# yml-bit/CTA-GAN

Hardware: AMD Instinct MI355X
Metric: paired 512x512 slices/sec (G+D step); generator rel-L2 vs CPU reference (higher is better)
Workload: dtype bf16; 1 GPU; HdGan stage-2 full G+D train step (G, Reg, STN, D_m, losses, Adam x3), 16 paired 512x512 slices/GPU; per_gpu_batch=16, global_batch=16, size=512, parallelism=single, rccl_ranks=1, dp_backend=none

## Files before the change

### cta_gan_amd/csrc/conv_dispatch.h

```cpp
#pragma once
#include "common.h"
#include "ctg_knobs.h"

static inline int tap_dy(int tw) { return (tw & 0xff) - 64; }
static inline int tap_dx(int tw) { return ((tw >> 8) & 0xff) - 64; }

struct TapWindow {
    int dymin = 127, dymax = -128, dxmin = 127, dxmax = -128;
    void add(int dy, int dx) {
        dymin = dy < dymin ? dy : dymin; dymax = dy > dymax ? dy : dymax;
        dxmin = dx < dxmin ? dx : dxmin; dxmax = dx > dxmax ? dx : dxmax;
    }
    int kh() const { return dymax - dymin + 1; }
    int kw() const { return dxmax - dxmin + 1; }
    int dy0() const { return dymin; }
    int dx0() const { return dxmin; }
};
static inline TapWindow tap_window(const int* taps, int ntaps) {
    TapWindow w;
    for (int t = 0; t < ntaps; ++t) w.add(tap_dy(taps[t]), tap_dx(taps[t]));
    return w;
}

static inline bool taps_3x3(const int* taps, bool flipped) {
    for (int t = 0; t < 9; ++t) {
        const int dy = t / 3 - 1, dx = t % 3 - 1;
        if (tap_dy(taps[t]) != (flipped ? -dy : dy) || tap_dx(taps[t]) != (flipped ? -dx : dx)) return false;
    }
    return true;
}
static inline bool taps_conv3x3_s2(const int* taps) {
    for (int t = 0; t < 9; ++t)
        if ((taps[t] >> 16) != t) return false;
    return taps_3x3(taps, false);
}
static inline bool taps_convT3x3_classes(const int* c_ntaps, const int* c_oy0, const int* c_ox0, const int* c_tap0, const int* taps) {
    static const int want_n[4] = {1, 2, 2, 4}, want_oy[4] = {0, 0, 1, 1}, want_ox[4] = {0, 1, 0, 1};
    static const int want_t[9][3] = {{0, 0, 4}, {0, 1, 3}, {0, 0, 5}, {1, 0, 1}, {0, 0, 7}, {1, 1, 0}, {1, 0, 2}, {0, 1, 6}, {0, 0, 8}};
    int t = 0;
    for (int q = 0; q < 4; ++q) {
        if (c_ntaps[q] != want_n[q] || c_oy0[q] != want_oy[q] || c_ox0[q] != want_ox[q] || c_tap0[q] != t) return false;
        for (int k = 0; k < want_n[q]; ++k, ++t)
            if (tap_dy(taps[t]) != want_t[t][0] || tap_dx(taps[t]) != want_t[t][1] || (taps[t] >> 16) != want_t[t][2]) return false;
    }
    return true;
}

struct BandPlan { int band_rows, nbands; };
static inline BandPlan band_plan(int rows, int min_band, long slots, long strips, int band_env) {
    long nb = slots / strips;
    if (nb < 1) nb = 1;
    int band = (int)((rows + nb - 1) / nb);
    if (band < min_band) band = min_band;
    if (band_env >= 8) band = band_env;
    return BandPlan{band, (rows + band - 1) / band};
}

template <auto Kernel, typename Args>
static int launch_lds(dim3 grid, dim3 block, int smem, hipStream_t st, const Args& s) {
    static unsigned long long attr_mask = 0;
    const int rc = ctg_lds_attr_once((const void*)Kernel, smem, &attr_mask);
    if (rc != CTG_OK) return rc;
    hipLaunchKernelGGL(Kernel, grid, block, smem, st, s);
    return ctg_launch_status();
}

static inline bool halo_th8(int Hs, int Ws, int Cout, int B, int ncls) {
    const long wgs = (long)((Hs + 15) / 16) * ((Ws + 15) / 16) * ((Cout + 127) / 128) * B;
    return !ctg_knobs().no_th8 && ncls != 4 && Hs >= 16 && wgs < ctg_knobs().th8_wgs;
}
```

### cta_gan_amd/csrc/conv_halo.h

```cpp
#pragma once
#include <stdlib.h>
#include <type_traits>
#include "common.h"
#include "conv_dispatch.h"

struct ConvArgs {
    const void* x;
    const void* w;
    void* y;
    const float* bias;
    int B, Hi, Wi, Cin, x_ld;
    int Ho, Wo, Cout, y_ld;
    int Hs, Ws, oy0, ox0, os, is;
    int frame;
    int pad_mode, act;
    int w_tap_stride;
    int ntaps;
    int taps[64];
    int kh, kw, dy0, dx0;
    float* stats;
    const void* res;
    const void* fold;
    int res_ld, fold_ld;
    const void* bz;
    const float* bmean;
    const float* brstd;
    float* bstats;
    int bz_ld, bact;
    int ncls;
    int s2d;
    int pair_lo;
    unsigned long long* nie_sync;
    int nie_act;
    int nie_budget;
    int c_ntaps[4], c_tap0[4], c_oy0[4], c_ox0[4], c_kh[4], c_kw[4], c_dy0[4], c_dx0[4];
};

typedef const __attribute__((address_space(1))) void* gptr_t;
typedef __attribute__((address_space(3))) void* lptr_t;

extern __device__ __attribute__((aligned(16))) unsigned g_zero_chunk[4];

__device__ __forceinline__ void unpack_bf16x8(const u32x4 t, float (&f)[8]) {
#pragma unroll
    for (int i = 0; i < 4; ++i) {
        f[2 * i] = __uint_as_float(t[i] << 16);
        f[2 * i + 1] = __uint_as_float(t[i] & 0xffff0000u);
    }
}
__device__ __forceinline__ void add_bf16x8(float (&f)[8], const bf16_t* p) {
    const u32x4 t = *reinterpret_cast<const u32x4*>(p);
#pragma unroll
    for (int i = 0; i < 4; ++i) {
        f[2 * i] += __uint_as_float(t[i] << 16);
        f[2 * i + 1] += __uint_as_float(t[i] & 0xffff0000u);
    }
}

#define CONV_ACT_RT (-1)
template <int ACT> __device__ __forceinline__ float act_apply_c(float x, int act) {
    if constexpr (ACT == ACT_NONE) return x;
    else if constexpr (ACT == ACT_RELU) return x > 0.f ? x : 0.f;
    else if constexpr (ACT == ACT_LRELU) return x > 0.f ? x : LRELU_SLOPE * x;
    else return act_apply(x, act);
}
template <typename F> __device__ __forceinline__ void act_switch(int act, F&& f) {
    if (act == ACT_NONE) f(std::integral_constant<int, ACT_NONE>{});
    else if (act == ACT_RELU) f(std::integral_constant<int, ACT_RELU>{});
    else if (act == ACT_LRELU) f(std::integral_constant<int, ACT_LRELU>{});
    else f(std::integral_constant<int, CONV_ACT_RT>{});
}
struct GradMask {
    float slope;
    unsigned keep;
    __device__ __forceinline__ explicit GradMask(int bact)
        : slope(bact == ACT_LRELU ? LRELU_SLOPE : 1.f), keep(bact == ACT_RELU ? 0u : 0xffffffffu) {}
    __device__ __forceinline__ float apply(float g, float xh) const {
        return xh > 0.f ? g : __uint_as_float(__float_as_uint(slope * g) & keep);
    }
};

template <int N, bool V1_FIRST> __device__ __forceinline__ float pinned_sumsq(const float (&v)[N]) {
#pragma clang fp contract(off)
    if constexpr (N == 1) {
        return v[0] * v[0];
    } else {
        float s = V1_FIRST ? __fmaf_rn(v[0], v[0], v[1] * v[1]) : __fmaf_rn(v[1], v[1], v[0] * v[0]);
#pragma unroll
        for (int k = 2; k < N; ++k) s = __fmaf_rn(v[k], v[k], s);
        return s;
    }
}

#define HALO_W 16

template <typename T, typename OutT, int BN, int WM, int WN, int KCH, int ABUF, int TH, bool FUSE, int KWC, bool MC = false, bool PK = false,
          bool S2D = false, bool NIE = false>
__global__ __launch_bounds__(WM * WN * 64, ((TH / WM) * (BN / (WN * 16)) > 16 ? 2 : 4))
void conv_halo_kernel(const ConvArgs a) {
    static_assert(!NIE || (!MC && !S2D && sizeof(T) == 2 && !std::is_same<OutT, float>::value),
                  "InstanceNorm in the epilogue: plain bf16 / split-pair launches");
    static_assert(!S2D || (!MC && !FUSE && KWC == 0 && ABUF == 1), "polyphase K walk: plain single-buffer instantiations");
    static_assert(!PK || (KCH == 8 && sizeof(T) == 2), "split-pair K steps: [hi 32 | lo 32] rows of bf16");
    constexpr int NTH = WM * WN * 64;
    constexpr int EPC = VecOf<T>::N;
    constexpr int BKE = KCH * EPC;
    constexpr int BM = TH * HALO_W;
    constexpr int TM = TH / WM;
    static_assert(TH % WM == 0, "tile rows per wave");
    constexpr int TN = BN / (WN * 16);
    constexpr int B_CH = BN * KCH;
    constexpr int B_IT = (B_CH + NTH - 1) / NTH;
    static_assert(B_CH % 64 == 0, "weight tile");
    extern __shared__ __attribute__((aligned(16))) char smem[];

    const int tid = threadIdx.x, lane = tid & 63, wave = __builtin_amdgcn_readfirstlane(tid >> 6);
    const int wm = wave / WN, wn = wave % WN;
    const int n = blockIdx.y;
    const int ntn = (a.Cout + BN - 1) / BN;
    const int id = xcd_contiguous(blockIdx.x, gridDim.x);
    const int n0 = (id % ntn) * BN;
    const int spc = id / ntn;
    int sp = spc, kh_ = a.kh, kw_ = a.kw, dy0 = a.dy0, dx0 = a.dx0, ntaps = a.ntaps, tap0 = 0, oy0_ = a.oy0, ox0_ = a.ox0;
    if constexpr (MC) {
        const int q = spc & 3;
        sp = spc >> 2;
        kh_ = a.c_kh[q]; kw_ = a.c_kw[q]; dy0 = a.c_dy0[q]; dx0 = a.c_dx0[q];
        ntaps = a.c_ntaps[q]; tap0 = a.c_tap0[q]; oy0_ = a.c_oy0[q]; ox0_ = a.c_ox0[q];
    }
    const int HPW = KWC ? HALO_W + KWC - 1 : HALO_W + kw_ - 1, HPH = TH + kh_ - 1;
    const int HPC = HPH * HPW * KCH;
    const int HPC64 = (HPC + 63) & ~63;
    const int nchunk = a.Cin / BKE;
    const int nbufA = (nchunk > 1 && ABUF == 2) ? 2 : 1;
    char* sA = smem;
    char* sB = smem + nbufA * HPC64 * 16;

    const int tx_n = (a.Ws + HALO_W - 1) / HALO_W;
    const int y0 = (sp / tx_n) * TH, x0 = (sp % tx_n) * HALO_W;
    const T* __restrict__ X = (const T*)a.x + (size_t)n * a.Hi * a.Wi * a.x_ld;
    const T* __restrict__ W = (const T*)a.w;

    const int h_it = (HPC64 + NTH - 1) / NTH;
    const unsigned hpw_magic = (unsigned)((0x100000000ULL + HPW - 1) / HPW);
    const int Hi = a.Hi, Wi = a.Wi, x_ld = a.x_ld, pad_mode = a.pad_mode;
    const int iy00 = y0 + dy0, ix00 = x0 + dx0;
    constexpr bool PRE = (KWC >= 3) && !MC;
    constexpr int H_PRE = PRE ? ((((TH + KWC - 1) * (HALO_W + KWC - 1) * KCH + 63) & ~63) + NTH - 1) / NTH : 1;
    int hoff[H_PRE];
    if constexpr (PRE) {
#pragma unroll
        for (int it = 0; it < H_PRE; ++it) {
            const int sl = tid + NTH * it;
            const int hrow = sl / KCH;
            const int hy = (int)__umulhi((unsigned)hrow, hpw_magic), hx = hrow - hy * HPW;
            const int kc = swz<KCH>(hx, sl % KCH);
            int iy = iy00 + hy, ix = ix00 + hx;
            if (pad_mode == PAD_REFLECT) {
                iy = reflect_idx(iy, Hi);
                ix = reflect_idx(ix, Wi);
            }
            const bool ok = (sl < HPC) && ((unsigned)iy < (unsigned)Hi) && ((unsigned)ix < (unsigned)Wi);
            hoff[it] = ok ? (iy * Wi + ix) * x_ld + (PK ? (kc & 3) * EPC + (kc >> 2) * a.pair_lo : kc * EPC) : -1;
        }
    }
    int phy = S2D ? a.c_oy0[0] : 0, phx = S2D ? a.c_ox0[0] : 0;
    auto issue_halo = [&](int it, int buf, int kc0) __attribute__((always_inline)) {
        if constexpr (PRE) {
#pragma unroll
            for (int j = 0; j < H_PRE; ++j) {
                if (j == it && NTH * j + 64 * wave < HPC64) {
                    const T* src = hoff[j] >= 0 ? X + (hoff[j] + kc0) : (const T*)g_zero_chunk;
                    __builtin_amdgcn_global_load_lds((gptr_t)src, (lptr_t)(sA + (buf * HPC64 + NTH * j + 64 * wave) * 16), 16, 0, 0);
                }
            }
        } else
        if (NTH * it + 64 * wave < HPC64) {
            const int sl = tid + NTH * it;
            const int hrow = sl / KCH;
            const int hy = (int)__umulhi((unsigned)hrow, hpw_magic), hx = hrow - hy * HPW;
            const int kc = swz<KCH>(hx, sl % KCH);
            int iy = iy00 + hy, ix = ix00 + hx;
            if constexpr (S2D) { iy = 2 * iy + phy; ix = 2 * ix + phx; }
            if (pad_mode == PAD_REFLECT) {
                iy = reflect_idx(iy, Hi);
                ix = reflect_idx(ix, Wi);
            }
            const bool ok = (sl < HPC) && ((unsigned)iy < (unsigned)Hi) && ((unsigned)ix < (unsigned)Wi);
            const T* src = ok ? X + ((iy * Wi + ix) * x_ld + (PK ? (kc & 3) * EPC + (kc >> 2) * a.pair_lo : kc * EPC) + kc0)
                              : (const T*)g_zero_chunk;
            __builtin_amdgcn_global_load_lds((gptr_t)src, (lptr_t)(sA + (buf * HPC64 + NTH * it + 64 * wave) * 16), 16, 0, 0);
        }
    };
    int boff[B_IT];
    const bool b_active = (B_CH % NTH == 0) || (tid < B_CH);
#pragma unroll
    for (int it = 0; it < B_IT; ++it) {
        const int s = (tid + NTH * it) % B_CH;
        const int row = s / KCH;
        boff[it] = (n0 + row) * a.Cin + swz<KCH>(row, s % KCH) * EPC;
    }
    const int w_tap_stride = a.w_tap_stride;
    auto issue_w = [&](int buf, int tw, int kc0) __attribute__((always_inline)) {
        if (b_active) {
            const int wbase = (tw >> 16) * w_tap_stride + kc0;
#pragma unroll
            for (int it = 0; it < B_IT; ++it)
                if (B_CH % NTH == 0 || NTH * it + 64 * wave < B_CH)
                    __builtin_amdgcn_global_load_lds((gptr_t)(W + wbase + boff[it]),
                                                     (lptr_t)(sB + (buf * B_CH + NTH * it + 64 * wave) * 16), 16, 0, 0);
        }
    };

    f32x4 acc[TM][TN];
#pragma unroll
    for (int i = 0; i < TM; ++i)
#pragma unroll
        for (int j = 0; j < TN; ++j) acc[i][j] = f32x4{0.f, 0.f, 0.f, 0.f};

    const int wo0 = (((wn * TN) * 16 + (lane & 15)) * KCH + swz<KCH>(lane & 15, lane >> 4)) * 16;
    auto compute = [&](int abuf, int bbuf, int tw) __attribute__((always_inline)) {
        const char* pa = sA + abuf * HPC64 * 16;
        const char* pb = sB + bbuf * B_CH * 16;
        const int ky = (tw & 0xff) - 64 - dy0, kx = ((tw >> 8) & 0xff) - 64 - dx0;
        const int hx = kx + (lane & 15);
        const char* prow = pa + (ky + wm * TM) * (HPW * KCH * 16);
        const int xo0 = (hx * KCH + swz<KCH>(hx, lane >> 4)) * 16;
        if constexpr (PK) {
            u32x4 fa[TM], fb[TN], fl[TN];
#pragma unroll
            for (int mt = 0; mt < TM; ++mt) fa[mt] = *reinterpret_cast<const u32x4*>(prow + xo0 + mt * (HPW * KCH * 16));
#pragma unroll
            for (int nt = 0; nt < TN; ++nt) fb[nt] = *reinterpret_cast<const u32x4*>(pb + wo0 + nt * (16 * KCH * 16));
#pragma unroll
            for (int mt = 0; mt < TM; ++mt)
#pragma unroll
                for (int nt = 0; nt < TN; ++nt)
                    acc[mt][nt] = __builtin_amdgcn_mfma_f32_16x16x32_bf16(
                        __builtin_bit_cast(bf16x8, fb[nt]), __builtin_bit_cast(bf16x8, fa[mt]), acc[mt][nt], 0, 0, 0);
#pragma unroll
            for (int nt = 0; nt < TN; ++nt) fl[nt] = *reinterpret_cast<const u32x4*>(pb + (wo0 ^ 64) + nt * (16 * KCH * 16));
#pragma unroll
            for (int mt = 0; mt < TM; ++mt)
#pragma unroll
                for (int nt = 0; nt < TN; ++nt)
                    acc[mt][nt] = __builtin_amdgcn_mfma_f32_16x16x32_bf16(
                        __builtin_bit_cast(bf16x8, fl[nt]), __builtin_bit_cast(bf16x8, fa[mt]), acc[mt][nt], 0, 0, 0);
#pragma unroll
            for (int mt = 0; mt < TM; ++mt) fa[mt] = *reinterpret_cast<const u32x4*>(prow + (xo0 ^ 64) + mt * (HPW * KCH * 16));
#pragma unroll
            for (int mt = 0; mt < TM; ++mt)
#pragma unroll
                for (int nt = 0; nt < TN; ++nt)
                    acc[mt][nt] = __builtin_amdgcn_mfma_f32_16x16x32_bf16(
                        __builtin_bit_cast(bf16x8, fb[nt]), __builtin_bit_cast(bf16x8, fa[mt]), acc[mt][nt], 0, 0, 0);
        } else
#pragma unroll
        for (int ks = 0; ks < KCH / 4; ++ks) {
            u32x4 fa[TM], fb[TN];
            const int xo = xo0 ^ (ks * 64), wo = wo0 ^ (ks * 64);
#pragma unroll
            for (int mt = 0; mt < TM; ++mt)
                fa[mt] = *reinterpret_cast<const u32x4*>(prow + xo + mt * (HPW * KCH * 16));
#pragma unroll
            for (int nt = 0; nt < TN; ++nt)
                fb[nt] = *reinterpret_cast<const u32x4*>(pb + wo + nt * (16 * KCH * 16));
#pragma unroll
            for (int mt = 0; mt < TM; ++mt)
#pragma unroll
                for (int nt = 0; nt < TN; ++nt) {
                    if constexpr (sizeof(T) == 2) {
                        acc[mt][nt] = __builtin_amdgcn_mfma_f32_16x16x32_bf16(
                            __builtin_bit_cast(bf16x8, fb[nt]), __builtin_bit_cast(bf16x8, fa[mt]), acc[mt][nt], 0, 0, 0);
                    } else {
                        const f32x4 va = __builtin_bit_cast(f32x4, fa[mt]);
                        const f32x4 vb = __builtin_bit_cast(f32x4, fb[nt]);
#pragma unroll
                        for (int q = 0; q < 4; ++q)
                            acc[mt][nt] = __builtin_amdgcn_mfma_f32_16x16x4f32(vb[q], va[q], acc[mt][nt], 0, 0, 0);
                    }
                }
        }
    };

    const bool wave_rows_valid = y0 + wm * TM < a.Hs;
    const int pps = (h_it + ntaps - 1) / ntaps;
    auto issue_halo_all = [&](int buf, int kc0) __attribute__((always_inline)) {
        if constexpr (PRE) {
#pragma unroll
            for (int j = 0; j < H_PRE; ++j)
                if (NTH * j + 64 * wave < HPC64) {
                    const T* src = hoff[j] >= 0 ? X + (hoff[j] + kc0) : (const T*)g_zero_chunk;
                    __builtin_amdgcn_global_load_lds((gptr_t)src, (lptr_t)(sA + (buf * HPC64 + NTH * j + 64 * wave) * 16), 16, 0, 0);
                }
        } else {
            for (int it = 0; it < h_it; ++it) issue_halo(it, buf, kc0);
        }
    };
    auto xslice = [&](int cc) __attribute__((always_inline)) { return PK ? cc * (BKE / 2) : cc * BKE; };
    if constexpr (S2D) { ntaps = a.c_ntaps[0]; tap0 = a.c_tap0[0]; }
    issue_halo_all(0, 0);
    int tw_cur = a.taps[tap0];
    issue_w(0, tw_cur, 0);
    __syncthreads();
    int S = nchunk * ntaps;
    if constexpr (S2D) {
        S = 0;
        for (int q = 0; q < a.ncls; ++q) S += nchunk * a.c_ntaps[q];
    }
    const int nslices = S2D ? nchunk * a.ncls : nchunk;
    int c = 0, t = 0;
    for (int s = 0; s < S; ++s) {
        int tn = t + 1, cn = c;
        if (tn == ntaps) { tn = 0; cn = c + 1; }
        int tw_next = 0;
        int ntaps_n = ntaps, tap0_n = tap0;
        if constexpr (S2D) {
            if (cn != c && cn < nslices) { const int q = cn / nchunk; ntaps_n = a.c_ntaps[q]; tap0_n = a.c_tap0[q]; }
        }
        if (s + 1 < S) {
            tw_next = a.taps[tap0_n + tn];
            issue_w((s + 1) & 1, tw_next, (S2D ? cn % nchunk : cn) * BKE);
        }
        if (ABUF == 2 && c + 1 < nchunk) {
            for (int q = 0; q < pps; ++q) {
                const int it = t * pps + q;
                if (it < h_it) issue_halo(it, (c + 1) & 1, xslice(c + 1));
            }
        }
        if (wave_rows_valid) compute(nbufA == 2 ? (c & 1) : 0, s & 1, tw_cur);
        __syncthreads();
        if (ABUF == 1 && cn != c && cn < nslices) {
            if constexpr (S2D) { const int q = cn / nchunk; phy = a.c_oy0[q]; phx = a.c_ox0[q]; }
            issue_halo_all(0, xslice(S2D ? cn % nchunk : cn));
            __syncthreads();
        }
        t = tn;
        c = cn;
        ntaps = ntaps_n;
        tap0 = tap0_n;
        tw_cur = tw_next;
    }

    const int co_l = (lane >> 4) * 4;
    if (a.stats != nullptr) {
        float* red = reinterpret_cast<float*>(smem);
#pragma unroll
        for (int nt = 0; nt < TN; ++nt) {
            float s1[4] = {0.f, 0.f, 0.f, 0.f}, s2[4], vq[4][TM];
#pragma unroll
            for (int mt = 0; mt < TM; ++mt) {
                const bool valid = (y0 + wm * TM + mt < a.Hs) && (x0 + (lane & 15) < a.Ws);
#pragma unroll
                for (int r = 0; r < 4; ++r) {
                    const float v = valid ? acc[mt][nt][r] : 0.f;
                    s1[r] += v;
                    vq[r][mt] = v;
                }
            }
#pragma unroll
            for (int r = 0; r < 4; ++r) s2[r] = pinned_sumsq<TM, KWC == 3 && !(FUSE && std::is_same<OutT, bfpair_t>::value)>(vq[r]);
#pragma unroll
            for (int r = 0; r < 4; ++r) {
                s1[r] = row16_sum_to_lane15(s1[r]);
                s2[r] = row16_sum_to_lane15(s2[r]);
                if ((lane & 15) == 15) {
                    const int cl = (wn * TN + nt) * 16 + co_l + r;
                    red[(wm * BN + cl) * 2] = s1[r];
                    red[(wm * BN + cl) * 2 + 1] = s2[r];
                }
            }
        }
        __syncthreads();
        const int ntile = gridDim.x / ntn;
        for (int cl = tid; cl < BN; cl += NTH) {
            if (n0 + cl < a.Cout) {
                float t1 = 0.f, t2 = 0.f;
#pragma unroll
                for (int w = 0; w < WM; ++w) { t1 += red[(w * BN + cl) * 2]; t2 += red[(w * BN + cl) * 2 + 1]; }
                float* dst = a.stats + (((size_t)n * ntile + spc) * a.Cout + n0 + cl) * 2;
                if constexpr (NIE) {
                    __hip_atomic_store(reinterpret_cast<unsigned long long*>(dst),
                                       (unsigned long long)__float_as_uint(t1) | ((unsigned long long)__float_as_uint(t2) << 32),
                                       __ATOMIC_RELAXED, __HIP_MEMORY_SCOPE_AGENT);
                } else {
                    dst[0] = t1;
                    dst[1] = t2;
                }
            }
        }
        __syncthreads();
    }
    float nmr[NIE ? TN : 1][4], nrr[NIE ? TN : 1][4];
    if constexpr (NIE) {
        int* s_ok = reinterpret_cast<int*>(smem);
        float* smr = reinterpret_cast<float*>(smem + 64);
        double* dred = reinterpret_cast<double*>(smem + 64 + BN * 8);
        const int ntile = gridDim.x / ntn;
        unsigned long long* cnt = a.nie_sync + 1 + (n * ntn + n0 / BN);
        asm volatile("s_waitcnt vmcnt(0)" ::: "memory");
        __syncthreads();
        if (tid == 0) {
            const unsigned long long old = __hip_atomic_fetch_add(cnt, 1ull, __ATOMIC_RELAXED, __HIP_MEMORY_SCOPE_AGENT);
            const unsigned long long target = (old / (unsigned)ntile + 1ull) * (unsigned)ntile;
            int budget = a.nie_budget;
            while (__hip_atomic_load(cnt, __ATOMIC_RELAXED, __HIP_MEMORY_SCOPE_AGENT) < target && --budget > 0)
                __builtin_amdgcn_s_sleep(8);
            *s_ok = budget > 0;
            if (budget <= 0) __hip_atomic_store(a.nie_sync, 1ull, __ATOMIC_RELAXED, __HIP_MEMORY_SCOPE_AGENT);
        }
        __syncthreads();
        const bool ok = *s_ok != 0;
        {
            static_assert(NTH % BN == 0, "finalize: whole channel rounds");
            constexpr int QS = NTH / BN;
            const int q = tid / BN, cl = tid % BN;
            double t1 = 0.0, t2 = 0.0;
            for (int s0 = q; s0 < ntile; s0 += 8 * QS) {
                unsigned long long v[8];
#pragma unroll
                for (int j = 0; j < 8; ++j) {
                    const int sl = s0 + j * QS;
                    const unsigned long long* p = reinterpret_cast<const unsigned long long*>(
                        a.stats + (((size_t)n * ntile + (sl < ntile ? sl : q)) * a.Cout + n0 + cl) * 2);
                    v[j] = __hip_atomic_load(p, __ATOMIC_RELAXED, __HIP_MEMORY_SCOPE_AGENT);
                }
#pragma unroll
                for (int j = 0; j < 8; ++j)
                    if (s0 + j * QS < ntile) {
                        t1 += (double)__uint_as_float((unsigned)(v[j] & 0xffffffffull));
                        t2 += (double)__uint_as_float((unsigned)(v[j] >> 32));
                    }
            }
            dred[(q * BN + cl) * 2] = t1;
            dred[(q * BN + cl) * 2 + 1] = t2;
            __syncthreads();
            if (tid < BN) {
                double u1 = 0.0, u2 = 0.0;
#pragma unroll
                for (int qq = 0; qq < QS; ++qq) { u1 += dred[(qq * BN + tid) * 2]; u2 += dred[(qq * BN + tid) * 2 + 1]; }
                const double inv = 1.0 / ((double)a.Hs * (double)a.Ws);
                const double m = u1 * inv;
                double var = u2 * inv - m * m;
                var = var < 0.0 ? 0.0 : var;
                const float nan = __uint_as_float(0x7fc00000u);
                smr[2 * tid] = ok ? (float)m : nan;
                smr[2 * tid + 1] = ok ? (float)(1.0 / sqrt(var + (double)IN_EPS)) : nan;
            }
            __syncthreads();
        }
#pragma unroll
        for (int nt = 0; nt < TN; ++nt)
#pragma unroll
            for (int r = 0; r < 4; ++r) {
                nmr[nt][r] = smr[2 * ((wn * TN + nt) * 16 + co_l + r)];
                nrr[nt][r] = smr[2 * ((wn * TN + nt) * 16 + co_l + r) + 1];
            }
        __syncthreads();
    }
    const int epi_act = NIE ? a.nie_act : a.act;
    if constexpr (std::is_same<OutT, bfpair_t>::value) {
        constexpr int NR = TN >= 4 ? 2 : 1;
        static_assert(WN == 1 || TN >= 4, "pair epilogue: the host sizes the staging tile for BN / WN channels");
        constexpr int TNR = TN / NR;
        constexpr int CR = WN * TNR * 16;
        constexpr int RS = CR * 4 + 16;
        constexpr int CPR = CR / 8;
        constexpr int NIT = BM * CPR / NTH;
        static_assert(BM * CPR % NTH == 0 && NTH % CPR == 0, "pair epilogue: whole trips, a thread keeps its channel chunk");
        char* st = smem;
        bf16_t* __restrict__ Y = (bf16_t*)a.y;
        const bf16_t* __restrict__ R = (const bf16_t*)a.res;
        const bf16_t* __restrict__ F = (const bf16_t*)a.fold;
        const bf16_t* __restrict__ Z = (const bf16_t*)a.bz;
        const bool bst = FUSE && a.bstats != nullptr;
        const GradMask bmask(a.bact);
        const int y_lo = a.y_ld >> 1, r_lo = a.res_ld >> 1, f_lo = a.fold_ld >> 1, z_lo = a.bz_ld >> 1;
        auto chan_of = [&](int col, int rd) __attribute__((always_inline)) {
            const int blk = col >> 4;
            return ((blk / TNR) * TN + rd * TNR + blk % TNR) * 16 + (col & 15);
        };
#pragma unroll
        for (int rd = 0; rd < NR; ++rd) {
            if (rd) __syncthreads();
            act_switch(epi_act, [&](auto AC) __attribute__((always_inline)) {
                constexpr int ACT = decltype(AC)::value;
#pragma unroll
                for (int ntl = 0; ntl < TNR; ++ntl) {
                    const int nt = rd * TNR + ntl;
                    const int co = (wn * TN + nt) * 16 + co_l;
                    float bv[4];
#pragma unroll
                    for (int r = 0; r < 4; ++r)
                        bv[r] = (a.bias != nullptr && n0 + co + r < a.Cout) ? a.bias[n0 + co + r] : 0.f;
#pragma unroll
                    for (int mt = 0; mt < TM; ++mt) {
                        const int prow = (wm * TM + mt) * HALO_W + (lane & 15);
                        f32x4 o;
#pragma unroll
                        for (int r = 0; r < 4; ++r) {
                            if constexpr (NIE) o[r] = act_apply_c<ACT>((acc[mt][nt][r] - nmr[nt][r]) * nrr[nt][r], epi_act);
                            else o[r] = act_apply_c<ACT>(acc[mt][nt][r] + bv[r], epi_act);
                        }
                        *reinterpret_cast<f32x4*>(st + prow * RS + ((wn * TNR + ntl) * 16 + co_l) * 4) = o;
                    }
                }
            });
            __syncthreads();
            const int chl = chan_of((tid % CPR) * 8, rd);
            float bs1[8], bs2[8], bmu[8], brs[8];
#pragma unroll
            for (int e = 0; e < 8; ++e) { bs1[e] = 0.f; bs2[e] = 0.f; bmu[e] = 0.f; brs[e] = 0.f; }
            if constexpr (FUSE) {
                if (bst && n0 + chl < a.Cout) {
#pragma unroll
                    for (int e = 0; e < 8; ++e) {
                        bmu[e] = a.bmean[(size_t)n * a.Cout + n0 + chl + e];
                        brs[e] = a.brstd[(size_t)n * a.Cout + n0 + chl + e];
                    }
                }
            }
#pragma unroll
            for (int it = 0; it < NIT; ++it) {
                const int cidx = tid + NTH * it;
                const int prow = cidx / CPR;
                const int oy = y0 + prow / HALO_W, ox = x0 + prow % HALO_W;
                if (oy < a.Hs && ox < a.Ws && n0 + chl < a.Cout) {
                    float f[8];
                    {
                        const f32x4 v0 = *reinterpret_cast<const f32x4*>(st + prow * RS + (tid % CPR) * 32);
                        const f32x4 v1 = *reinterpret_cast<const f32x4*>(st + prow * RS + (tid % CPR) * 32 + 16);
#pragma unroll
                        for (int e = 0; e < 4; ++e) { f[e] = v0[e]; f[4 + e] = v1[e]; }
                    }
                    if constexpr (FUSE) {
                        if (R != nullptr) {
                            const bf16_t* rp = R + (((size_t)n * a.Hs + oy) * a.Ws + ox) * a.res_ld + n0 + chl;
                            add_bf16x8(f, rp);
                            add_bf16x8(f, rp + r_lo);
                        }
                        if (F != nullptr) {
                            const int ey = oy == 1 ? 0 : (oy == a.Hs - 2 ? a.Hs + 1 : -1);
                            const int ex = ox == 1 ? 0 : (ox == a.Ws - 2 ? a.Ws + 1 : -1);
                            const bf16_t* Fn = F + (size_t)n * (a.Hs + 2) * (a.Ws + 2) * a.fold_ld + n0 + chl;
                            if (ey >= 0) {
                                const bf16_t* q = Fn + ((size_t)ey * (a.Ws + 2) + ox + 1) * a.fold_ld;
                                add_bf16x8(f, q); add_bf16x8(f, q + f_lo);
                            }
                            if (ex >= 0) {
                                const bf16_t* q = Fn + ((size_t)(oy + 1) * (a.Ws + 2) + ex) * a.fold_ld;
                                add_bf16x8(f, q); add_bf16x8(f, q + f_lo);
                            }
                            if (ey >= 0 && ex >= 0) {
                                const bf16_t* q = Fn + ((size_t)ey * (a.Ws + 2) + ex) * a.fold_ld;
                                add_bf16x8(f, q); add_bf16x8(f, q + f_lo);
                            }
                        }
                    }
                    bf16x8 hi, lo;
#pragma unroll
                    for (int e = 0; e < 8; ++e) {
                        hi[e] = (bf16_t)f[e];
                        lo[e] = (bf16_t)(f[e] - (float)hi[e]);
                    }
                    bf16_t* yp = Y + (((size_t)n * a.Ho + (oy * a.os + oy0_)) * a.Wo + (ox * a.os + ox0_)) * a.y_ld + n0 + chl;
                    *reinterpret_cast<bf16x8*>(yp) = hi;
                    *reinterpret_cast<bf16x8*>(yp + y_lo) = lo;
                    if constexpr (FUSE) {
                        if (bst) {
                            const bf16_t* zp = Z + (((size_t)n * a.Hs + oy) * a.Ws + ox) * a.bz_ld + n0 + chl;
                            float zf[8];
#pragma unroll
                            for (int e = 0; e < 8; ++e) zf[e] = 0.f;
                            add_bf16x8(zf, zp);
                            add_bf16x8(zf, zp + z_lo);
#pragma unroll
                            for (int e = 0; e < 8; ++e) {
                                const float xh = (zf[e] - bmu[e]) * brs[e];
                                const float gg = bmask.apply((float)hi[e] + (float)lo[e], xh);
                                bs1[e] += gg;
                                bs2[e] += gg * xh;
                            }
                        }
                    }
                }
            }
            if constexpr (FUSE) {
                if (bst) {
                    __syncthreads();
                    float* red = reinterpret_cast<float*>(smem);
#pragma unroll
                    for (int e = 0; e < 8; ++e) { red[tid * 16 + e] = bs1[e]; red[tid * 16 + 8 + e] = bs2[e]; }
                    __syncthreads();
                    const int ntile = gridDim.x / ntn;
                    for (int cl = tid; cl < CR; cl += NTH) {
                        const int ch = chan_of(cl, rd);
                        if (n0 + ch < a.Cout) {
                            float t1 = 0.f, t2 = 0.f;
                            for (int q = 0; q < NTH / CPR; ++q) {
                                const float* r = red + (q * CPR + (cl >> 3)) * 16 + (cl & 7);
                                t1 += r[0];
                                t2 += r[8];
                            }
                            float* dst = a.bstats + (((size_t)n * ntile + spc) * a.Cout + n0 + ch) * 2;
                            dst[0] = t1;
                            dst[1] = t2;
                        }
                    }
                }
            }
        }
    } else if constexpr (sizeof(OutT) == 2) {
        constexpr int RS = BN * 2 + 16;
        char* st = smem;
        act_switch(epi_act, [&](auto AC) __attribute__((always_inline)) {
            constexpr int ACT = decltype(AC)::value;
#pragma unroll
            for (int nt = 0; nt < TN; ++nt) {
                const int co = (wn * TN + nt) * 16 + co_l;
                float bv[4];
#pragma unroll
                for (int r = 0; r < 4; ++r)
                    bv[r] = (a.bias != nullptr && n0 + co + r < a.Cout) ? a.bias[n0 + co + r] : 0.f;
#pragma unroll
                for (int mt = 0; mt < TM; ++mt) {
                    const int prow = (wm * TM + mt) * HALO_W + (lane & 15);
                    bf16x4 o;
#pragma unroll
                    for (int r = 0; r < 4; ++r) {
                        if constexpr (NIE) o[r] = (bf16_t)act_apply_c<ACT>((acc[mt][nt][r] - nmr[nt][r]) * nrr[nt][r], epi_act);
                        else o[r] = (bf16_t)act_apply_c<ACT>(acc[mt][nt][r] + bv[r], epi_act);
                    }
                    *reinterpret_cast<bf16x4*>(st + prow * RS + co * 2) = o;
                }
            }
        });
        OutT* __restrict__ Y = (OutT*)a.y;
        const bf16_t* __restrict__ R = (const bf16_t*)a.res;
        const bf16_t* __restrict__ F = (const bf16_t*)a.fold;
        constexpr int CPR = BN / 8;
        constexpr int NIT = BM * CPR / NTH;
        constexpr int RPT = NTH / (CPR * HALO_W);
        static_assert(NTH % (CPR * HALO_W) == 0 && (CPR * HALO_W) % 64 == 0, "store loop: whole tile rows per trip, one row per wave");
        const int ch = (tid % CPR) * 8;
        const int prow0 = tid / CPR;
        const int oyb = y0 + __builtin_amdgcn_readfirstlane(tid / (CPR * HALO_W)), ox = x0 + prow0 % HALO_W;
        const bool col_ok = ox < a.Ws && n0 + ch < a.Cout;
        OutT* const yp0 = Y + (((size_t)n * a.Ho + (oyb * a.os + oy0_)) * a.Wo + (ox * a.os + ox0_)) * a.y_ld + n0 + ch;
        const size_t y_step = (size_t)RPT * a.os * a.Wo * a.y_ld;
        const size_t pix0 = ((size_t)n * a.Hs + oyb) * a.Ws + ox;
        const bf16_t* const zero16 = (const bf16_t*)g_zero_chunk;
        u32x4 rv[FUSE ? NIT : 1], zv[FUSE ? NIT : 1];
        if constexpr (FUSE) {
            const bf16_t* const rp0 = R + pix0 * a.res_ld + n0 + ch;
            const bf16_t* const zp0 = (const bf16_t*)a.bz + pix0 * a.bz_ld + n0 + ch;
            const size_t r_step = (size_t)RPT * a.Ws * a.res_ld, z_step = (size_t)RPT * a.Ws * a.bz_ld;
#pragma unroll
            for (int it = 0; it < NIT; ++it) {
                const bool in = col_ok && oyb + RPT * it < a.Hs;
                rv[it] = *reinterpret_cast<const u32x4*>(R != nullptr && in ? rp0 + it * r_step : zero16);
                zv[it] = *reinterpret_cast<const u32x4*>(a.bstats != nullptr && in ? zp0 + it * z_step : zero16);
            }
        }
        bool fold_tile = false;
        const bf16_t* fn0 = zero16;
        size_t f_pitch = 0;
        int ex = -1;
        u32x4 fcol = {};
        auto fold_ey = [&](int it) __attribute__((always_inline)) {
            const int oy = oyb + RPT * it;
            return oy >= a.Hs ? -1 : (oy == 1 ? 0 : (oy == a.Hs - 2 ? a.Hs + 1 : -1));
        };
        auto fold_col_request = [&](int it) __attribute__((always_inline)) {
            const bool colf = col_ok && ex >= 0 && oyb + RPT * it < a.Hs;
            fcol = *reinterpret_cast<const u32x4*>(colf ? fn0 + (size_t)(oyb + RPT * it + 1) * f_pitch + (size_t)ex * a.fold_ld : zero16);
        };
        if constexpr (FUSE) {
            if (F != nullptr) {
                const int yl = min(y0 + TH, a.Hs), xl = min(x0 + HALO_W, a.Ws);
                fold_tile = (y0 <= 1 && 1 < yl) || (y0 <= a.Hs - 2 && a.Hs - 2 < yl) || (x0 <= 1 && 1 < xl) || (x0 <= a.Ws - 2 && a.Ws - 2 < xl);
            }
            if (fold_tile) {
                fn0 = F + (size_t)n * (a.Hs + 2) * (a.Ws + 2) * a.fold_ld + n0 + ch;
                f_pitch = (size_t)(a.Ws + 2) * a.fold_ld;
                ex = ox == 1 ? 0 : (ox == a.Ws - 2 ? a.Ws + 1 : -1);
                fold_col_request(0);
            }
        }
        const bool bst = FUSE && a.bstats != nullptr;
        float bs1[8], bs2[8], bmu[8], brs[8];
#pragma unroll
        for (int e = 0; e < 8; ++e) { bs1[e] = 0.f; bs2[e] = 0.f; bmu[e] = 0.f; brs[e] = 0.f; }
        if constexpr (FUSE) {
            if (bst && n0 + ch < a.Cout) {
#pragma unroll
                for (int e = 0; e < 8; ++e) {
                    bmu[e] = a.bmean[(size_t)n * a.Cout + n0 + ch + e];
                    brs[e] = a.brstd[(size_t)n * a.Cout + n0 + ch + e];
                }
            }
        }
        __syncthreads();
        const GradMask bmask(a.bact);
        const char* const sp0 = st + prow0 * RS + ch * 2;
#pragma unroll
        for (int it = 0; it < NIT; ++it) {
            if (oyb + RPT * it < a.Hs && col_ok) {
                if constexpr (FUSE) {
                    u32x4 v = *reinterpret_cast<const u32x4*>(sp0 + it * (RPT * HALO_W * RS));
                    float f[8], g[8];
                    unpack_bf16x8(v, f);
                    unpack_bf16x8(rv[it], g);
#pragma unroll
                    for (int e = 0; e < 8; ++e) f[e] += g[e];
                    if (fold_tile) {
                        const int ey = fold_ey(it);
                        if (ey >= 0) add_bf16x8(f, fn0 + (size_t)ey * f_pitch + (size_t)(ox + 1) * a.fold_ld);
                        if (ex >= 0) {
                            unpack_bf16x8(fcol, g);
#pragma unroll
                            for (int e = 0; e < 8; ++e) f[e] += g[e];
                        }
                        if (ey >= 0 && ex >= 0) add_bf16x8(f, fn0 + (size_t)ey * f_pitch + (size_t)ex * a.fold_ld);
                        if (it + 1 < NIT) fold_col_request(it + 1);
                    }
                    bf16x8 o;
#pragma unroll
                    for (int e = 0; e < 8; ++e) o[e] = (bf16_t)f[e];
                    if (bst) {
                        float zf[8];
                        unpack_bf16x8(zv[it], zf);
#pragma unroll
                        for (int e = 0; e < 8; ++e) {
                            const float xh = (zf[e] - bmu[e]) * brs[e];
                            const float gg = bmask.apply((float)o[e], xh);
                            bs1[e] += gg;
                            bs2[e] += gg * xh;
                        }
                    }
                    *reinterpret_cast<u32x4*>(yp0 + it * y_step) = __builtin_bit_cast(u32x4, o);
                } else {
                    *reinterpret_cast<u32x4*>(yp0 + it * y_step) = *reinterpret_cast<const u32x4*>(sp0 + it * (RPT * HALO_W * RS));
                }
            }
        }
        if constexpr (FUSE) {
            if (bst) {
                __syncthreads();
                float* red = reinterpret_cast<float*>(smem);
#pragma unroll
                for (int e = 0; e < 8; ++e) { red[tid * 16 + e] = bs1[e]; red[tid * 16 + 8 + e] = bs2[e]; }
                __syncthreads();
                const int ntile = gridDim.x / ntn;
                for (int cl = tid; cl < BN; cl += NTH) {
                    if (n0 + cl < a.Cout) {
                        float t1 = 0.f, t2 = 0.f;
                        for (int q = 0; q < NTH / CPR; ++q) {
                            const float* r = red + (q * CPR + (cl >> 3)) * 16 + (cl & 7);
                            t1 += r[0];
                            t2 += r[8];
                        }
                        float* dst = a.bstats + (((size_t)n * ntile + spc) * a.Cout + n0 + cl) * 2;
                        dst[0] = t1;
                        dst[1] = t2;
                    }
                }
            }
        }
    } else {
        OutT* __restrict__ Y = (OutT*)a.y;
        const bool vec_ok = ((a.Cout & 3) == 0) && ((a.y_ld & 3) == 0);
        OutT* const yp0 = Y + (((size_t)n * a.Ho + ((y0 + wm * TM) * a.os + oy0_)) * a.Wo + ((x0 + (lane & 15)) * a.os + ox0_)) * a.y_ld;
        const size_t y_step = (size_t)a.os * a.Wo * a.y_ld;
        auto store_rows = [&](auto AC) __attribute__((always_inline)) {
        constexpr int ACT = decltype(AC)::value;
#pragma unroll
        for (int mt = 0; mt < TM; ++mt) {
            const int oy = y0 + wm * TM + mt, ox = x0 + (lane & 15);
            if (oy >= a.Hs || ox >= a.Ws) continue;
            OutT* yp = yp0 + mt * y_step;
#pragma unroll
            for (int nt = 0; nt < TN; ++nt) {
                const int co = n0 + (wn * TN + nt) * 16 + co_l;
                if (co >= a.Cout) continue;
                float v[4];
#pragma unroll
                for (int r = 0; r < 4; ++r) {
                    const float b = (a.bias != nullptr && co + r < a.Cout) ? a.bias[co + r] : 0.f;
                    v[r] = act_apply_c<ACT>(acc[mt][nt][r] + b, epi_act);
                }
                if (FUSE && a.res != nullptr) {
                    const float* rp = (const float*)a.res + (((size_t)n * a.Hs + oy) * a.Ws + ox) * a.res_ld + co;
#pragma unroll
                    for (int r = 0; r < 4; ++r)
                        if (co + r < a.Cout) v[r] += rp[r];
                }
                if (FUSE && a.fold != nullptr) {
                    const int ey = oy == 1 ? 0 : (oy == a.Hs - 2 ? a.Hs + 1 : -1);
                    const int ex = ox == 1 ? 0 : (ox == a.Ws - 2 ? a.Ws + 1 : -1);
                    const float* Fn = (const float*)a.fold + (size_t)n * (a.Hs + 2) * (a.Ws + 2) * a.fold_ld + co;
#pragma unroll
                    for (int r = 0; r < 4; ++r) {
                        if (co + r >= a.Cout) continue;
                        if (ey >= 0) v[r] += Fn[((size_t)ey * (a.Ws + 2) + ox + 1) * a.fold_ld + r];
                        if (ex >= 0) v[r] += Fn[((size_t)(oy + 1) * (a.Ws + 2) + ex) * a.fold_ld + r];
                        if (ey >= 0 && ex >= 0) v[r] += Fn[((size_t)ey * (a.Ws + 2) + ex) * a.fold_ld + r];
                    }
                }
                if (vec_ok) {
                    *reinterpret_cast<f32x4*>(yp + co) = f32x4{v[0], v[1], v[2], v[3]};
                } else {
#pragma unroll
                    for (int r = 0; r < 4; ++r)
                        if (co + r < a.Cout) yp[co + r] = v[r];
                }
            }
        }
        };
        if constexpr (FUSE) store_rows(std::integral_constant<int, CONV_ACT_RT>{});
        else act_switch(epi_act, store_rows);
    }
}

template <typename T, typename OutT, int BN, int WM, int WN, int KCH, int ABUF, int TH = 16, bool FUSE = false, int KWC = 0, bool MC = false, bool PK = false,
          bool S2D = false, bool NIE = false>
static int launch_halo_cfg(const ConvArgs& a, hipStream_t st, int* tiles_out = nullptr) {
    if constexpr (!NIE && KWC == 3 && (TH == 16 || (TH == 8 && !PK)) && BN == 128 && WM == 4 && WN == 2 && KCH == 8 && !MC && !S2D &&
                  sizeof(T) == 2 && ((std::is_same<OutT, bf16_t>::value && !PK) || (std::is_same<OutT, bfpair_t>::value && PK))) {
        if (a.nie_sync != nullptr) {
            if ((FUSE && (a.fold != nullptr || a.bstats != nullptr)) || a.stats == nullptr || a.Cout % BN) return CTG_EINVAL;
            return launch_halo_cfg<T, OutT, BN, WM, WN, KCH, ABUF, TH, FUSE, KWC, false, PK, false, true>(a, st, tiles_out);
        }
    }
    if constexpr (!S2D && !FUSE && !MC && KWC == 0 && TH == 16 && sizeof(T) == 2 && KCH == 8 && BN >= 64 && !std::is_same<OutT, float>::value) {
        if (a.s2d) {
            if (a.res != nullptr || a.fold != nullptr) return -1;
            return launch_halo_cfg<T, OutT, BN, WM, WN, KCH, ABUF, TH, false, 0, false, PK, true>(a, st, tiles_out);
        }
    }
    if (a.s2d && !S2D) return -1;
    if constexpr (!FUSE && !MC && !S2D && !NIE) {
        if (a.res != nullptr || a.fold != nullptr) return launch_halo_cfg<T, OutT, BN, WM, WN, KCH, ABUF, TH, true, KWC, false, PK>(a, st, tiles_out);
    }
    if constexpr (!MC && !S2D && !FUSE && KWC == 0 && (TH == 16 || (TH == 8 && BN == 64)) && sizeof(T) == 2 &&
                  ((std::is_same<OutT, bf16_t>::value && !PK) || (std::is_same<OutT, bfpair_t>::value && PK))) {
        if (a.ncls == 4) return launch_halo_cfg<T, OutT, BN, WM, WN, KCH, ABUF, TH, false, 0, true, PK>(a, st, tiles_out);
    }
    if constexpr (KWC == 0 && !MC && !S2D && sizeof(T) == 2) {
        if (a.kw == 3 && a.kh <= 3 && a.ncls <= 1) return launch_halo_cfg<T, OutT, BN, WM, WN, KCH, ABUF, TH, FUSE, 3, false, PK>(a, st, tiles_out);
    }
    if (a.ncls > 1 && !MC && !S2D) return -1;
    if (a.nie_sync != nullptr && !NIE) return CTG_EINVAL;
    constexpr int NTH = WM * WN * 64;
    const int hpw = HALO_W + a.kw - 1, hph = TH + a.kh - 1;
    const int hpc = hph * hpw * KCH;
    const int hpc64 = (hpc + 63) & ~63;
    const int epc = VecOf<T>::N;
    const int nchunk = a.Cin / (KCH * epc);
    const int main_lds = (((nchunk > 1 && ABUF == 2) ? 2 : 1) * hpc64 + 2 * BN * KCH) * 16;
    const int epi_lds = std::is_same<OutT, bfpair_t>::value ? TH * HALO_W * ((BN / WN) * 4 + 16)
                        : sizeof(OutT) == 2 ? TH * HALO_W * (BN * 2 + 16) : 0;
    if (FUSE && a.bstats != nullptr && WM * WN * 64 * 64 > (main_lds > epi_lds ? main_lds : epi_lds)) return -1;
    const int smem = main_lds > epi_lds ? main_lds : epi_lds;
    if (smem > 160 * 1024 || hph * hpw >= 65536) return -1;
    static unsigned long long attr_mask = 0;
    {
        const int rc = ctg_lds_attr_once((const void*)conv_halo_kernel<T, OutT, BN, WM, WN, KCH, ABUF, TH, FUSE, KWC, MC, PK, S2D, NIE>,
                                         160 * 1024, &attr_mask);
        if (rc != CTG_OK) return rc;
    }
    const int tiles = ((a.Hs + TH - 1) / TH) * ((a.Ws + HALO_W - 1) / HALO_W) * (MC ? 4 : 1);
    if (tiles_out != nullptr) *tiles_out = tiles;
    const int ntn = (a.Cout + BN - 1) / BN;
    if constexpr (NIE) {
        static int occ_dev[64];
        int dev = 0;
        if (hipGetDevice(&dev) != hipSuccess) dev = 0;
        dev &= 63;
        if (occ_dev[dev] == 0) {
            int occ = 0;
            if (hipOccupancyMaxActiveBlocksPerMultiprocessor(
                    &occ, (const void*)conv_halo_kernel<T, OutT, BN, WM, WN, KCH, ABUF, TH, FUSE, KWC, MC, PK, S2D, NIE>, NTH, smem) != hipSuccess ||
                occ < 1)
                occ = 1;
            occ_dev[dev] = occ;
        }
        const int share = ctg_knobs().nie_share > 0 ? ctg_knobs().nie_share : 2;
        if ((long)tiles * ntn * share > (long)occ_dev[dev] * ctg_cu_count()) return 2;
    }
    dim3 grid(tiles * ntn, a.B);
    hipLaunchKernelGGL((conv_halo_kernel<T, OutT, BN, WM, WN, KCH, ABUF, TH, FUSE, KWC, MC, PK, S2D, NIE>), grid, dim3(NTH), smem, st, a);
    return ctg_launch_status();
}

static int launch_strip32(const ConvArgs& a, hipStream_t st, int* tiles_out, bool pair);

template <typename T, int KCH>
static int launch_halo_t(const ConvArgs& a, int out_f32, hipStream_t st, int* tiles_out) {
    if (a.is != 1 && !a.s2d) return -1;
    if (out_f32 >= 2) {
        if constexpr (sizeof(T) == 2 && KCH == 8) {
            if (out_f32 == 2) {
                if (a.Cout > 64) return launch_halo_cfg<T, bfpair_t, 128, 4, 2, 8, 1, 16, false, 0, false, true>(a, st, tiles_out);
                if (a.Cout > 32) {
                    if (a.ncls == 4 && !ctg_knobs().no_mc_th8) return launch_halo_cfg<T, bfpair_t, 64, 4, 1, 8, 1, 8, false, 0, false, true>(a, st, tiles_out);
                    if (!ctg_knobs().no_th8_64 && a.ncls <= 1 && a.Hs >= 16)
                        return launch_halo_cfg<T, bfpair_t, 64, 4, 1, 8, 1, 8, false, 0, false, true>(a, st, tiles_out);
                    return launch_halo_cfg<T, bfpair_t, 64, 4, 1, 8, 1, 16, false, 0, false, true>(a, st, tiles_out);
                }
                if (a.Cout > 16) {
                    const int rc = launch_strip32(a, st, tiles_out, true);
                    if (rc != -1) return rc;
                    return launch_halo_cfg<T, bfpair_t, 32, 4, 1, 8, 1, 16, false, 0, false, true>(a, st, tiles_out);
                }
                return -1;
            }
            if (a.Cout > 64) return launch_halo_cfg<T, float, 128, 4, 2, 8, 1, 16, false, 0, false, true>(a, st, tiles_out);
            if (a.Cout > 32) return launch_halo_cfg<T, float, 64, 4, 1, 8, 1, 16, false, 0, false, true>(a, st, tiles_out);
            if (a.Cout > 16) return launch_halo_cfg<T, float, 32, 4, 1, 8, 1, 16, false, 0, false, true>(a, st, tiles_out);
            return launch_halo_cfg<T, float, 16, 4, 1, 8, 1, 16, false, 0, false, true>(a, st, tiles_out);
        }
        return -1;
    }
    if (a.Cout > 64) {
        if (out_f32) {
            if constexpr (sizeof(T) == 2) return launch_halo_cfg<T, float, 128, 4, 2, KCH, 1>(a, st, tiles_out);
            return -1;
        }
        if constexpr (sizeof(T) == 2) {
            static_assert(HALO_W == 16, "halo_th8 counts 16-column tiles");
            if (halo_th8(a.Hs, a.Ws, a.Cout, a.B, a.ncls)) return launch_halo_cfg<T, T, 128, 4, 2, KCH, 1, 8>(a, st, tiles_out);
        }
        return launch_halo_cfg<T, T, 128, 4, 2, KCH, 1>(a, st, tiles_out);
    }
    if (a.Cout > 32) {
        if (out_f32) {
            if constexpr (sizeof(T) == 2) return launch_halo_cfg<T, float, 64, 4, 1, KCH, 1>(a, st, tiles_out);
            return -1;
        }
        if constexpr (sizeof(T) == 2 && KCH == 8) {
            if (!ctg_knobs().no_th8_64 && (a.ncls <= 1 || a.ncls == 4) && a.Hs >= 16) return launch_halo_cfg<T, T, 64, 4, 1, KCH, 1, 8>(a, st, tiles_out);
        }
        return launch_halo_cfg<T, T, 64, 4, 1, KCH, 1>(a, st, tiles_out);
    }
    if (a.Cout > 16) {
        if (out_f32) {
            if constexpr (sizeof(T) == 2) return launch_halo_cfg<T, float, 32, 4, 1, KCH, 1>(a, st, tiles_out);
            return -1;
        }
        if constexpr (sizeof(T) == 2 && KCH == 4) {
            const int rc = launch_strip32(a, st, tiles_out, false);
            if (rc != -1) return rc;
        }
        return launch_halo_cfg<T, T, 32, 4, 1, KCH, 1>(a, st, tiles_out);
    }
    if (out_f32 || sizeof(T) == 4) return launch_halo_cfg<T, float, 16, 4, 1, KCH, 1>(a, st, tiles_out);
    return -1;
}
```

Before: 337.1 slices/s.

## Add fully unrolled 3x3 tap-walk main loop for single-buffered halo conv

Adds a specialised main loop for 3x3 convolutions (forward or flipped taps) in the single-buffered, non-packed bf16 halo kernel. It unrolls the nine taps at compile time, advances the weight pointer incrementally, precomputes the LDS fragment offsets and double-buffers weight loads between taps. The aim is to cut the per-tap scalar work of the generic loop: tap decoding, index arithmetic and branching. The host checks the tap pattern and sets a walk3 flag. Compile-time unrolling increases code size and register pressure, and asm barriers are used to pin the schedule.

```diff
diff --git a/cta_gan_amd/csrc/conv_dispatch.h b/cta_gan_amd/csrc/conv_dispatch.h
--- a/cta_gan_amd/csrc/conv_dispatch.h
+++ b/cta_gan_amd/csrc/conv_dispatch.h
@@ -28,6 +28,17 @@
         if (tap_dy(taps[t]) != (flipped ? -dy : dy) || tap_dx(taps[t]) != (flipped ? -dx : dx)) return false;
     }
     return true;
+}
+static inline int taps_3x3_walk(const int* taps, int ntaps, int kh, int kw, int dy0, int dx0) {
+    if (ntaps != 9 || kh != 3 || kw != 3) return 0;
+    bool fwd = true, flip = true;
+    for (int t = 0; t < 9; ++t) {
+        if ((taps[t] >> 16) != t) return 0;
+        const int ky = tap_dy(taps[t]) - dy0, kx = tap_dx(taps[t]) - dx0;
+        fwd = fwd && ky == t / 3 && kx == t % 3;
+        flip = flip && ky == 2 - t / 3 && kx == 2 - t % 3;
+    }
+    return fwd ? 1 : (flip ? 2 : 0);
 }
 static inline bool taps_conv3x3_s2(const int* taps) {
     for (int t = 0; t < 9; ++t)
diff --git a/cta_gan_amd/csrc/conv_halo.h b/cta_gan_amd/csrc/conv_halo.h
--- a/cta_gan_amd/csrc/conv_halo.h
+++ b/cta_gan_amd/csrc/conv_halo.h
@@ -18,6 +18,7 @@
     int ntaps;
     int taps[64];
     int kh, kw, dy0, dx0;
+    int walk3;
     float* stats;
     const void* res;
     const void* fold;
@@ -219,13 +220,7 @@
         for (int j = 0; j < TN; ++j) acc[i][j] = f32x4{0.f, 0.f, 0.f, 0.f};
 
     const int wo0 = (((wn * TN) * 16 + (lane & 15)) * KCH + swz<KCH>(lane & 15, lane >> 4)) * 16;
-    auto compute = [&](int abuf, int bbuf, int tw) __attribute__((always_inline)) {
-        const char* pa = sA + abuf * HPC64 * 16;
-        const char* pb = sB + bbuf * B_CH * 16;
-        const int ky = (tw & 0xff) - 64 - dy0, kx = ((tw >> 8) & 0xff) - 64 - dx0;
-        const int hx = kx + (lane & 15);
-        const char* prow = pa + (ky + wm * TM) * (HPW * KCH * 16);
-        const int xo0 = (hx * KCH + swz<KCH>(hx, lane >> 4)) * 16;
+    auto mma_tap = [&](const char* prow, int xo0, const char* pb) __attribute__((always_inline)) {
         if constexpr (PK) {
             u32x4 fa[TM], fb[TN], fl[TN];
 #pragma unroll
@@ -281,6 +276,13 @@
                     }
                 }
         }
+    };
+    auto compute = [&](int abuf, int bbuf, int tw) __attribute__((always_inline)) {
+        const char* pa = sA + abuf * HPC64 * 16;
+        const char* pb = sB + bbuf * B_CH * 16;
+        const int ky = (tw & 0xff) - 64 - dy0, kx = ((tw >> 8) & 0xff) - 64 - dx0;
+        const int hx = kx + (lane & 15);
+        mma_tap(pa + (ky + wm * TM) * (HPW * KCH * 16), (hx * KCH + swz<KCH>(hx, lane >> 4)) * 16, pb);
     };
 
     const bool wave_rows_valid = y0 + wm * TM < a.Hs;
@@ -310,6 +312,74 @@
     }
     const int nslices = S2D ? nchunk * a.ncls : nchunk;
     int c = 0, t = 0;
+    constexpr bool WALK = KWC == 3 && ABUF == 1 && !MC && !S2D && !PK && sizeof(T) == 2;
+    bool walked = false;
+    if constexpr (WALK) {
+        static_assert(KCH == 4 || KCH == 8, "walk3x3: the row pitch keeps bit 6 of a fragment offset free");
+        constexpr int ROWP = (HALO_W + 2) * KCH * 16;
+        constexpr int HPC64_C = ((TH + 2) * (HALO_W + 2) * KCH + 63) & ~63;
+        constexpr int WT = B_CH * 16;
+        auto walk3x3 = [&](auto FL) __attribute__((always_inline)) {
+            constexpr bool FLIP = decltype(FL)::value;
+            int xa[3];
+#pragma unroll
+            for (int k = 0; k < 3; ++k) {
+                const int hx = k + (lane & 15);
+                xa[k] = (hx * KCH + swz<KCH>(hx, lane >> 4)) * 16 + wm * TM * ROWP;
+            }
+            const bool tail_mine = NTH * (H_PRE - 1) + 64 * wave < HPC64_C;
+            const T* zsrc = (const T*)g_zero_chunk;
+            asm volatile("" : "+s"(zsrc));
+            const char* sBc = smem + HPC64_C * 16;
+            const char* wp = reinterpret_cast<const char*>(W);
+            const long wstep = (long)w_tap_stride * (long)sizeof(T);
+            const long wwrap = (long)BKE * (long)sizeof(T) - 8 * wstep;
+            int wb0 = 0, wb1 = WT;
+            unsigned boffb[B_IT];
+#pragma unroll
+            for (int it = 0; it < B_IT; ++it) boffb[it] = (unsigned)boff[it] * (unsigned)sizeof(T);
+            for (int cc = 0; cc < nchunk; ++cc) {
+                const bool more = cc + 1 < nchunk;
+#pragma unroll
+                for (int tt = 0; tt < 9; ++tt) {
+                    if (tt < 8 || more) {
+                        wp += tt < 8 ? wstep : wwrap;
+                        if (b_active) {
+                            const int dst = ((tt + 1) & 1) ? wb1 : wb0;
+#pragma unroll
+                            for (int it = 0; it < B_IT; ++it)
+                                if (B_CH % NTH == 0 || NTH * it + 64 * wave < B_CH) {
+                                    asm volatile("" : "+v"(boffb[it]));
+                                    __builtin_amdgcn_global_load_lds((gptr_t)(wp + boffb[it]),
+                                                                     (lptr_t)(sBc + dst + (NTH * it + 64 * wave) * 16), 16, 0, 0);
+                                }
+                        }
+                    }
+                    __builtin_amdgcn_sched_barrier(0);
+                    if (wave_rows_valid) {
+                        const int ky = FLIP ? 2 - tt / 3 : tt / 3, kx = FLIP ? 2 - tt % 3 : tt % 3;
+                        mma_tap(smem + ky * ROWP, xa[kx], sBc + ((tt & 1) ? wb1 : wb0));
+                    }
+                    __syncthreads();
+                }
+                if (more) {
+                    int kc0 = xslice(cc + 1);
+                    asm volatile("" : "+s"(kc0));
+#pragma unroll
+                    for (int j = 0; j < H_PRE; ++j)
+                        if (NTH * (j + 1) <= HPC64_C || tail_mine) {
+                            const T* src = hoff[j] >= 0 ? X + (hoff[j] + kc0) : zsrc;
+                            __builtin_amdgcn_global_load_lds((gptr_t)src, (lptr_t)(smem + (NTH * j + 64 * wave) * 16), 16, 0, 0);
+                        }
+                    __syncthreads();
+                    const int w = wb0; wb0 = wb1; wb1 = w;
+                }
+            }
+        };
+        if (a.walk3 == 1) { walk3x3(std::false_type{}); walked = true; }
+        else if (a.walk3 == 2) { walk3x3(std::true_type{}); walked = true; }
+    }
+    if (!walked)
     for (int s = 0; s < S; ++s) {
         int tn = t + 1, cn = c;
         if (tn == ntaps) { tn = 0; cn = c + 1; }
@@ -889,7 +959,9 @@
         if ((long)tiles * ntn * share > (long)occ_dev[dev] * ctg_cu_count()) return 2;
     }
     dim3 grid(tiles * ntn, a.B);
-    hipLaunchKernelGGL((conv_halo_kernel<T, OutT, BN, WM, WN, KCH, ABUF, TH, FUSE, KWC, MC, PK, S2D, NIE>), grid, dim3(NTH), smem, st, a);
+    ConvArgs b = a;
+    b.walk3 = (KWC == 3 && ABUF == 1 && !MC && !S2D && !PK) ? taps_3x3_walk(a.taps, a.ntaps, a.kh, a.kw, a.dy0, a.dx0) : 0;
+    hipLaunchKernelGGL((conv_halo_kernel<T, OutT, BN, WM, WN, KCH, ABUF, TH, FUSE, KWC, MC, PK, S2D, NIE>), grid, dim3(NTH), smem, st, b);
     return ctg_launch_status();
 }
 
```

After: 342.9 slices/s, median of 6. 1.02x the previous value.
